# lorenzrichter/path-space-PDE-solver

Hardware: AMD Instinct MI355X
Metric: trajectory-timesteps/sec (K*N/s), d=100 HJB log-variance training iteration (higher is better)
Workload: dtype f32 (f16x3 split products: every matrix product as three f16 MFMAs, fp32 accumulate; state / sums fp32)

## Files before the change

### path-space-pde-solver_amd/csrc/hjb_kernels.h

```cpp
#pragma once
#include <cstdlib>
#include <type_traits>
#include <hip/hip_runtime.h>
#include <stdint.h>

namespace psp {

typedef float f32x4 __attribute__((ext_vector_type(4)));

struct HjbArgs {
    const float* params;
    const float* x0;
    const float* y0;
    const float* xi;
    float* path;
    float* D;
    float* XN;
    double* fwd_partial;
    const float* drift;
    const float* sigma;
    const float* runcost;
    const float* term;
    const double* sums;
    float* grad_partial;
// ... 91 lines not shown
    return addr;
}
template <class T>
__device__ __forceinline__ const T* opaque(const T* p) {
    return p + opaque_i(0);
}

#define PSP_PATH_STORE(ptr, val) __builtin_nontemporal_store((val), (ptr))

#ifndef PSP_PHILOX_ROUNDS
#define PSP_PHILOX_ROUNDS 7
#endif
constexpr int kPhiloxRounds = PSP_PHILOX_ROUNDS;
__device__ __forceinline__ void philox4x32_R(uint32_t c0, uint32_t c1, uint32_t c2, uint32_t c3,
                                             uint32_t k0, uint32_t k1, uint32_t (&out)[4]) {
#pragma unroll
    for (int r = 0; r < kPhiloxRounds; ++r) {
        const unsigned long long p0 = (unsigned long long)0xD2511F53u * (unsigned long long)c0;
        const unsigned long long p1 = (unsigned long long)0xCD9E8D57u * (unsigned long long)c2;
        const uint32_t hi0 = (uint32_t)(p0 >> 32), lo0 = (uint32_t)p0;
        const uint32_t hi1 = (uint32_t)(p1 >> 32), lo1 = (uint32_t)p1;
        const uint32_t n0 = __builtin_amdgcn_bitop3_b32(hi1, c1, k0, 0x96), n2 = __builtin_amdgcn_bitop3_b32(hi0, c3, k1, 0x96);
        c0 = n0; c1 = lo1; c2 = n2; c3 = lo0;
        k0 += 0x9E3779B9u; k1 += 0xBB67AE85u;
    }
    out[0] = c0; out[1] = c1; out[2] = c2; out[3] = c3;
}

__device__ __forceinline__ void philox_round(uint32_t& c0, uint32_t& c1, uint32_t& c2, uint32_t& c3, uint32_t k0, uint32_t k1) {
    const unsigned long long p0 = (unsigned long long)0xD2511F53u * (unsigned long long)c0;
    const unsigned long long p1 = (unsigned long long)0xCD9E8D57u * (unsigned long long)c2;
    const uint32_t hi0 = (uint32_t)(p0 >> 32), lo0 = (uint32_t)p0;
    const uint32_t hi1 = (uint32_t)(p1 >> 32), lo1 = (uint32_t)p1;
    const uint32_t n0 = __builtin_amdgcn_bitop3_b32(hi1, c1, k0, 0x96), n2 = __builtin_amdgcn_bitop3_b32(hi0, c3, k1, 0x96);
    c0 = n0; c1 = lo1; c2 = n2; c3 = lo0;
}

__device__ __forceinline__ f32x4 normal4(const uint32_t (&r)[4]) {
    const float s24 = 1.0f / 16777216.0f, h24 = 0.5f / 16777216.0f;
    const float u0 = __builtin_fmaf((float)(r[0] >> 8), s24, h24);
    const float u1 = __builtin_fmaf((float)(r[1] >> 8), s24, h24);
    const float u2 = __builtin_fmaf((float)(r[2] >> 8), s24, h24);
    const float u3 = __builtin_fmaf((float)(r[3] >> 8), s24, h24);
    const float ra = __builtin_amdgcn_sqrtf(-1.3862943611198906f * __builtin_amdgcn_logf(u0));
    const float rb = __builtin_amdgcn_sqrtf(-1.3862943611198906f * __builtin_amdgcn_logf(u2));
    f32x4 z;
    z[0] = ra * __builtin_amdgcn_cosf(u1);
    z[1] = ra * __builtin_amdgcn_sinf(u1);
    z[2] = rb * __builtin_amdgcn_cosf(u3);
    z[3] = rb * __builtin_amdgcn_sinf(u3);
    return z;
}

__device__ __forceinline__ f32x4 philox_block(uint32_t kglob, uint32_t step, uint32_t idx, uint32_t iter,
                                              uint32_t seed_lo, uint32_t seed_hi) {
    uint32_t r[4];
    philox4x32_R(kglob, step, idx, iter, seed_lo, seed_hi, r);
    return normal4(r);
}

template <int D, int DB>
__device__ __forceinline__ void regen_xi(f32x4 (&xin)[DB], uint32_t kglob, uint32_t n, int q, uint32_t iter,
                                         uint32_t seed_lo, uint32_t seed_hi) {
#pragma unroll
    for (int b = 0; b < DB; ++b) {
        xin[b] = philox_block(kglob, n, (uint32_t)(4 * b + q), iter, seed_lo, seed_hi);
        if (16 * b + 16 > D) {
#pragma unroll
            for (int r = 0; r < 4; ++r) if (16 * b + 4 * r + q >= D) xin[b][r] = 0.f;
        }
    }
}

template <class F>
__device__ __forceinline__ void stage_aop(float* dst, int MB, int KS, int tid, int nthr, F src) {
    const int total = MB * KS * 64;
    for (int idx = tid; idx < total; idx += nthr) {
        const int lane = idx & 63, t = idx >> 6;
        const int ks = t % KS, mb = t / KS;
        const int i = lane & 15, q = lane >> 4;
        dst[idx] = src(16 * mb + 4 * (i & 3) + (i >> 2), 4 * ks + q);
    }
}
template <class F>
__device__ __forceinline__ void stage_vec(float* dst, int NBLK, int tid, int nthr, F v) {
    for (int idx = tid; idx < NBLK * 16; idx += nthr) {
        const int r = idx & 3, q = (idx >> 2) & 3, b = idx >> 4;
        dst[idx] = v(16 * b + 4 * r + q);
    }
}

constexpr int kFenceMask = 0x1 | 0x2 | 0x4 | 0x10 | 0x20 | 0x40;
constexpr int kFenceAluOnly = 0x2 | 0x4;
template <int MB, int KS, int INB>
__device__ __forceinline__ void gemm_T(f32x4 (&acc)[MB], const float* wlds,
                                       const f32x4 (&in)[INB], int lane) {
    static_assert(INB * 4 >= KS, "input panel too small");
    static_assert(MB * KS * 256 <= 65536, "table exceeds the 16-bit ds_read immediate offset");
    constexpr int CH = (MB >= 4) ? 2 : 4;
    constexpr int NCH = cdiv(KS, CH);
    lane = opaque_i(lane);
    float buf[2][CH * MB];
#pragma unroll
    for (int kk = 0; kk < CH; ++kk)
#pragma unroll
        for (int mb = 0; mb < MB; ++mb)
// ... 159 lines not shown
#pragma unroll
            for (int e = 0; e < 8; ++e) {
                _Float16 h, l;
                split_f16(src(row, 32 * S + (e < 4 ? 4 * e : 16 + 4 * (e - 4)) + g), h, l);
                hi[e] = h; lo[e] = l;
            }
            f16x8* p = reinterpret_cast<f16x8*>(dstf + mb * SG::per_mb + S * 512);
            p[lane] = hi; p[64 + lane] = lo;
        }
    }
    if constexpr (SG::ODD) {
        for (int idx = tid; idx < MB * 64; idx += nthr) {
            const int lane = idx & 63, mb = idx >> 6;
            const int i = lane & 15, g = lane >> 4;
            const int row = 16 * mb + 4 * (i & 3) + (i >> 2);
            if constexpr (SG::ODD_F32) {
                dstf[mb * SG::per_mb + SG::NS * 512 + lane] = src(row, 32 * SG::NS + g);
            } else {
                f16x4 hi, lo;
#pragma unroll
                for (int e = 0; e < 4; ++e) {
                    _Float16 h, l;
                    split_f16(src(row, 32 * SG::NS + 4 * e + g), h, l);
                    hi[e] = h; lo[e] = l;
                }
                f16x4* p = reinterpret_cast<f16x4*>(dstf + mb * SG::per_mb + SG::NS * 512);
                p[lane] = hi; p[64 + lane] = lo;
            }
        }
    }
}
struct NoBetween { __device__ __forceinline__ void operator()(int) const {} };
template <int MB, int KS, int INB, int CU = 2, class BT = NoBetween>
__device__ __forceinline__ void gemm_Tx(f32x4 (&acc)[MB], const float* wlds, const f32x4 (&in)[INB], int lane, BT between = BT()) {
    constexpr int kFence = std::is_same<BT, NoBetween>::value ? kFenceMask : 0;
    using SG = SplitGeo<KS, INB>;
    constexpr int NS = SG::NS;
    static_assert(MB * SG::per_mb * 4 <= 65536, "table exceeds the 16-bit ds_read immediate offset");
    lane = opaque_i(lane);
    f32x4 corr[MB];
#pragma unroll
    for (int mb = 0; mb < MB; ++mb) corr[mb] = f32x4{0.f, 0.f, 0.f, 0.f};
    if constexpr (NS > 0) {
        const f16x8* tbl = reinterpret_cast<const f16x8*>(wlds) + lane;
        constexpr int NU = NS * MB, R = 2 * CU, PF = R - 1;
        f16x8 ah[R], al[R];
#pragma unroll
        for (int u = 0; u < PF; ++u)
            if (u < NU) {
                ah[u % R] = tbl[((u % MB) * SG::per_mb + (u / MB) * 512) / 4];
                al[u % R] = tbl[((u % MB) * SG::per_mb + (u / MB) * 512) / 4 + 64];
            }
        f16x8 bh, bl;
#pragma unroll
        for (int u = 0; u < NU; ++u) {
            if (u + PF < NU) {
                const int v = u + PF;
                ah[v % R] = tbl[((v % MB) * SG::per_mb + (v / MB) * 512) / 4];
                al[v % R] = tbl[((v % MB) * SG::per_mb + (v / MB) * 512) / 4 + 64];
            }
            const int S = u / MB, mb = u % MB;
            if (mb == 0) split8(in[2 * S], in[2 * S + 1], bh, bl);
            acc[mb] = __builtin_amdgcn_mfma_f32_16x16x32_f16(ah[u % R], bh, acc[mb], 0, 0, 0);
            corr[mb] = __builtin_amdgcn_mfma_f32_16x16x32_f16(ah[u % R], bl, corr[mb], 0, 0, 0);
            corr[mb] = __builtin_amdgcn_mfma_f32_16x16x32_f16(al[u % R], bh, corr[mb], 0, 0, 0);
            between(u);
            __builtin_amdgcn_sched_barrier(kFence);
        }
    }
    if constexpr (SG::ODD_F32) {
        const float bop = in[INB - 1][0];
#pragma unroll
        for (int mb = 0; mb < MB; ++mb) acc[mb] = mfma16(wlds[mb * SG::per_mb + NS * 512 + lane], bop, acc[mb]);
    }
    if constexpr (SG::ODD_H16) {
        f16x4 bh, bl;
        split4c(in[INB - 1], bh, bl);
#pragma unroll
        for (int mb = 0; mb < MB; ++mb) {
            const f16x4* p = reinterpret_cast<const f16x4*>(wlds + mb * SG::per_mb + NS * 512) + lane;
            const f16x4 a_hi = p[0], a_lo = p[64];
            acc[mb] = __builtin_amdgcn_mfma_f32_16x16x16f16(a_hi, bh, acc[mb], 0, 0, 0);
            corr[mb] = __builtin_amdgcn_mfma_f32_16x16x16f16(a_hi, bl, corr[mb], 0, 0, 0);
            corr[mb] = __builtin_amdgcn_mfma_f32_16x16x16f16(a_lo, bh, corr[mb], 0, 0, 0);
        }
    }
#pragma unroll
    for (int mb = 0; mb < MB; ++mb) acc[mb] = acc[mb] + kSplitInv * corr[mb];
}

template <int INB>
__device__ __forceinline__ void split_panel8(const f32x4 (&in)[INB], f16x8 (&bh)[INB / 2 > 0 ? INB / 2 : 1], f16x8 (&bl)[INB / 2 > 0 ? INB / 2 : 1]) {
#pragma unroll
    for (int S = 0; S < INB / 2; ++S) split8(in[2 * S], in[2 * S + 1], bh[S], bl[S]);
}
template <int MB, int KS, int INB, int CU = 2, class BT = NoBetween>
__device__ __forceinline__ void gemm_Txs(f32x4 (&acc)[MB], const float* wlds, const f16x8 (&bh)[INB / 2 > 0 ? INB / 2 : 1],
                                         const f16x8 (&bl)[INB / 2 > 0 ? INB / 2 : 1], const f32x4& last, int lane, BT between = BT()) {
    constexpr int kFence = std::is_same<BT, NoBetween>::value ? kFenceMask : 0;
    using SG = SplitGeo<KS, INB>;
    constexpr int NS = SG::NS;
    lane = opaque_i(lane);
    f32x4 corr[MB];
#pragma unroll
    for (int mb = 0; mb < MB; ++mb) corr[mb] = f32x4{0.f, 0.f, 0.f, 0.f};
    if constexpr (NS > 0) {
        const f16x8* tbl = reinterpret_cast<const f16x8*>(wlds) + lane;
        constexpr int NU = NS * MB, R = 2 * CU, PF = R - 1;
        f16x8 ah[R], al[R];
#pragma unroll
        for (int u = 0; u < PF; ++u)
            if (u < NU) {
                ah[u % R] = tbl[((u % MB) * SG::per_mb + (u / MB) * 512) / 4];
                al[u % R] = tbl[((u % MB) * SG::per_mb + (u / MB) * 512) / 4 + 64];
            }
#pragma unroll
        for (int u = 0; u < NU; ++u) {
            if (u + PF < NU) {
                const int v = u + PF;
                ah[v % R] = tbl[((v % MB) * SG::per_mb + (v / MB) * 512) / 4];
                al[v % R] = tbl[((v % MB) * SG::per_mb + (v / MB) * 512) / 4 + 64];
            }
            const int S = u / MB, mb = u % MB;
            acc[mb] = __builtin_amdgcn_mfma_f32_16x16x32_f16(ah[u % R], bh[S], acc[mb], 0, 0, 0);
            corr[mb] = __builtin_amdgcn_mfma_f32_16x16x32_f16(ah[u % R], bl[S], corr[mb], 0, 0, 0);
            corr[mb] = __builtin_amdgcn_mfma_f32_16x16x32_f16(al[u % R], bh[S], corr[mb], 0, 0, 0);
            between(u);
            __builtin_amdgcn_sched_barrier(kFence);
        }
    }
    if constexpr (SG::ODD_F32) {
        const float bop = last[0];
#pragma unroll
        for (int mb = 0; mb < MB; ++mb) acc[mb] = mfma16(wlds[mb * SG::per_mb + NS * 512 + lane], bop, acc[mb]);
    }
    if constexpr (SG::ODD_H16) {
        f16x4 b4h, b4l;
        split4c(last, b4h, b4l);
#pragma unroll
        for (int mb = 0; mb < MB; ++mb) {
            const f16x4* p = reinterpret_cast<const f16x4*>(wlds + mb * SG::per_mb + NS * 512) + lane;
            const f16x4 a_hi = p[0], a_lo = p[64];
            acc[mb] = __builtin_amdgcn_mfma_f32_16x16x16f16(a_hi, b4h, acc[mb], 0, 0, 0);
            corr[mb] = __builtin_amdgcn_mfma_f32_16x16x16f16(a_hi, b4l, corr[mb], 0, 0, 0);
            corr[mb] = __builtin_amdgcn_mfma_f32_16x16x16f16(a_lo, b4h, corr[mb], 0, 0, 0);
        }
    }
#pragma unroll
    for (int mb = 0; mb < MB; ++mb) acc[mb] = acc[mb] + kSplitInv * corr[mb];
}

__device__ __forceinline__ float qsum(float v) {
    v += __shfl_xor(v, 16);
    v += __shfl_xor(v, 32);
    return v;
}
__device__ __forceinline__ float jsumf(float v) {
    v += __shfl_xor(v, 1);
    v += __shfl_xor(v, 2);
    v += __shfl_xor(v, 4);
    v += __shfl_xor(v, 8);
    return v;
}
__device__ __forceinline__ double jsum(double v) {
    v += __shfl_xor(v, 1);
    v += __shfl_xor(v, 2);
    v += __shfl_xor(v, 4);
    v += __shfl_xor(v, 8);
    return v;
}

__device__ __forceinline__ float tanh_f32(float x) {
    const float e = __builtin_amdgcn_exp2f(fabsf(x) * 2.8853900817779268f);
    const float big = fmaf(-2.0f, __builtin_amdgcn_rcpf(e + 1.0f), 1.0f);
    return copysignf(big, x);
}
__device__ __forceinline__ f32x4 tanh4(f32x4 v) {
    f32x4 o;
    o[0] = tanh_f32(v[0]); o[1] = tanh_f32(v[1]); o[2] = tanh_f32(v[2]); o[3] = tanh_f32(v[3]);
    return o;
}
// ... 104 lines not shown
    const int k = t16 * 16 + j;
    const bool kvalid = wave_valid && k < a.K_local;
    const uint32_t kglob = (uint32_t)(a.k_offset + k);
    const float dt = a.dt, sqdt = a.sqdt;

    const float store_cxi = SPEC ? 1.f : ((k_store == 3) ? 0.f : 1.f);
    const float store_cz = SPEC ? 0.f : ((k_store == 3) ? 1.f : (k_store == 2 ? -a.sqdt : (k_adaptive ? 0.f : a.sqdt)));
    const bool do_store = FAST ? true : (k_store != 0);
    double sD = 0.0, sD2 = 0.0;
    if (wave_valid) {
        const f32x4* vecs0 = reinterpret_cast<const f32x4*>(lds + VEC) + q;
        const f32x4* vterm = vecs0 + (G::vterm - G::fVec) / 4;

        f32x4 X[DB];
#pragma unroll
        for (int b = 0; b < DB; ++b) {
#pragma unroll
            for (int r = 0; r < 4; ++r) {
                const int f = 16 * b + 4 * r + q;
                const float v = a.x0[(size_t)(kvalid ? k : 0) * a.x0_stride + (f < D ? f : D - 1)];
                X[b][r] = (f < D && kvalid) ? v : 0.f;
            }
        }
        float Y = a.y0 ? a.y0[0] : 0.f;
        float Fsum = 0.f, ULsum = 0.f;
#ifdef PSP_STAMPS
        unsigned long long stamps[8] = {0, 0, 0, 0, 0, 0, 0, 0};
#endif

        for (int n = 0; n < a.N; ++n) {
            PSP_STAMP(fs0);
            float tn = (float)n * dt;
            if constexpr (!FAST) { if (a.tfeat) tn = a.tfeat[n]; }
            const f32x4* vecs = opaque(vecs0);
            const f32x4* vb1 = vecs + (G::vb1 - G::fVec) / 4;
            const f32x4* vw1t = vecs + (G::vw1t - G::fVec) / 4;
            const f32x4* vb2 = vecs + (G::vb2 - G::fVec) / 4;
            const f32x4* vb3 = vecs + (G::vb3 - G::fVec) / 4;
            const f32x4* vdr = vecs + (G::vdr - G::fVec) / 4;
            const f32x4* vrun = vecs + (G::vrun - G::fVec) / 4;
            float* pblk = a.path + ((size_t)n * a.ntile16 + t16) * (size_t)G::PB + lane;
            auto x_store = [&](int u, int NU) __attribute__((always_inline)) {
                if (do_store) {
#pragma unroll
                    for (int ks = 0; ks < 4 * DB; ++ks)
                        if (ks >= u * (4 * DB) / NU && ks < (u + 1) * (4 * DB) / NU)
                            PSP_PATH_STORE(pblk + (G::pX / 64 + ks) * 64, X[ks >> 2][ks & 3]);
                }
            };
            if (!X3 && do_store) {
#pragma unroll
                for (int ks = 0; ks < 4 * DB; ++ks) PSP_PATH_STORE(pblk + (G::pX / 64 + ks) * 64, X[ks >> 2][ks & 3]);
            }
            f32x4 h1[HB];
#pragma unroll
            for (int m = 0; m < HB; ++m) h1[m] = vb1[m * 4] + tn * vw1t[m * 4];
            f32x4 Tn[DB];
            const bool early_drift = X3 && k_drift == DRIFT_DENSE;
            if constexpr (X3) {
                if (k_drift == DRIFT_DENSE) {
                    f16x8 xh[DB / 2 > 0 ? DB / 2 : 1], xl[DB / 2 > 0 ? DB / 2 : 1];
                    constexpr int NU1 = (DB / 2) * HB, NU2 = (DB / 2) * DB;
                    split_panel8<DB>(X, xh, xl);
                    gemm_Txs<HB, KSD, DB, 2>(h1, lds + oW1, xh, xl, X[DB - 1], lane, [&](int u) __attribute__((always_inline)) { x_store(u, NU1 + NU2); });
#pragma unroll
                    for (int b = 0; b < DB; ++b) Tn[b] = X[b];
                    gemm_Txs<DB, KSD, DB, 2>(Tn, ldsA, xh, xl, X[DB - 1], lane, [&](int u) __attribute__((always_inline)) { x_store(NU1 + u, NU1 + NU2); });
                    if constexpr (NU1 + NU2 == 0) x_store(0, 1);
                } else {
                    constexpr int NU1 = (DB / 2) * HB;
                    gemm_Tx<HB, KSD, DB, 2>(h1, lds + oW1, X, lane, [&](int u) __attribute__((always_inline)) { x_store(u, NU1); });
                    if constexpr (NU1 == 0) x_store(0, 1);
                }
            }
            else if constexpr (BF16) gemm_Tb<HB, DB>(h1, lds + oW1, X, lane);
            else gemm_T<HB, KSD, DB>(h1, lds + oW1, X, lane);
            PSP_STAMP(fs1);
#pragma unroll
            for (int m = 0; m < HB; ++m) h1[m] = tanh4(h1[m]);
            PSP_STAMP(fs2);
            f32x4 h2[HB];
#pragma unroll
            for (int m = 0; m < HB; ++m) h2[m] = vb2[m * 4];
            constexpr int NUH2 = (HB / 2) * HB, NUH3 = (HB / 2) * DB;
            constexpr bool PREGEN = X3 && FAST && (NUH2 + NUH3 > 0);
            [[maybe_unused]] f32x4 xig[PREGEN ? DB : 1];
            [[maybe_unused]] uint32_t pc0 = 0, pc1 = 0, pc2 = 0, pc3 = 0;
            constexpr int NSPC = kPhiloxRounds + 1;
            auto philox_slice = [&](int sidx) __attribute__((always_inline)) {
                const int b = sidx / NSPC, sub = sidx % NSPC;
                if (sub == 0) { pc0 = kglob; pc1 = (uint32_t)n; pc2 = (uint32_t)(4 * b + q); pc3 = iter_now; }
                if (sub < kPhiloxRounds) {
                    philox_round(pc0, pc1, pc2, pc3, a.seed_lo + (uint32_t)sub * 0x9E3779B9u, a.seed_hi + (uint32_t)sub * 0xBB67AE85u);
                    asm volatile("" : "+v"(pc0), "+v"(pc1), "+v"(pc2), "+v"(pc3));
                } else {
                    const uint32_t rr[4] = {pc0, pc1, pc2, pc3};
                    f32x4 xi = normal4(rr);
                    if (16 * b + 16 > D) {
#pragma unroll
                        for (int r = 0; r < 4; ++r) if (16 * b + 4 * r + q >= D) xi[r] = 0.f;
                    }
                    asm volatile("" : "+v"(xi));
                    xig[b < DB ? b : 0] = xi;
                }
            };
            auto philox_portion = [&](int u) __attribute__((always_inline)) {
                if constexpr (PREGEN) {
#pragma unroll
                    for (int sidx = 0; sidx < NSPC * DB; ++sidx)
                        if (sidx >= u * (NSPC * DB) / (NUH2 + NUH3) && sidx < (u + 1) * (NSPC * DB) / (NUH2 + NUH3)) philox_slice(sidx);
                }
            };
            auto h_store = [&](const f32x4 (&h)[HB], int slot, int u, int NU) __attribute__((always_inline)) {
                if (do_store) {
#pragma unroll
                    for (int ks = 0; ks < 4 * HB; ++ks)
                        if (ks >= u * (4 * HB) / NU && ks < (u + 1) * (4 * HB) / NU)
                            PSP_PATH_STORE(pblk + (slot / 64 + ks) * 64, h[ks >> 2][ks & 3]);
                }
            };
            if constexpr (X3) {
                gemm_Tx<HB, KSH, HB, 2>(h2, lds + oW2, h1, lane, [&](int u) __attribute__((always_inline)) { h_store(h1, G::pH1, u, NUH2); philox_portion(u); });
                if constexpr (NUH2 == 0) h_store(h1, G::pH1, 0, 1);
            }
            else if constexpr (BF16) gemm_Tb<HB, HB>(h2, lds + oW2, h1, lane);
            else gemm_T<HB, KSH, HB>(h2, lds + oW2, h1, lane);
#pragma unroll
            for (int m = 0; m < HB; ++m) h2[m] = tanh4(h2[m]);
            if (!X3 && do_store) {
#pragma unroll
                for (int ks = 0; ks < 4 * HB; ++ks) {
                    PSP_PATH_STORE(pblk + (G::pH1 / 64 + ks) * 64, h1[ks >> 2][ks & 3]);
                    PSP_PATH_STORE(pblk + (G::pH2 / 64 + ks) * 64, h2[ks >> 2][ks & 3]);
                }
            }
            f32x4 Z[DB];
#pragma unroll
            for (int m = 0; m < DB; ++m) Z[m] = vb3[m * 4];
            if constexpr (X3) {
                gemm_Tx<DB, KSH, HB, 2>(Z, lds + oW3, h2, lane, [&](int u) __attribute__((always_inline)) { h_store(h2, G::pH2, u, NUH3); philox_portion(NUH2 + u); });
                if constexpr (NUH3 == 0) h_store(h2, G::pH2, 0, 1);
            }
            else if constexpr (BF16) gemm_Tb<DB, HB>(Z, lds + oW3, h2, lane);
            else gemm_T<DB, KSH, HB>(Z, lds + oW3, h2, lane);
            PSP_STAMP(fs3);

            float S = 0.f, Pz = 0.f, UL = 0.f;
#pragma unroll
            for (int b = 0; b < DB; ++b) {
                f32x4 xi;
                if constexpr (PREGEN) {
                    xi = xig[b];
                } else if (FAST || a.noise_mode == NOISE_PHILOX) {
                    xi = philox_block(kglob, (uint32_t)n, (uint32_t)(4 * b + q), iter_now, a.seed_lo, a.seed_hi);
                } else {
                    const float* xrow = a.xi + ((size_t)(n + 1) * a.K_local + (kvalid ? k : 0)) * D;
#pragma unroll
                    for (int r = 0; r < 4; ++r) {
                        const int f = 16 * b + 4 * r + q;
                        const float v = xrow[f < D ? f : D - 1];
                        xi[r] = (f < D && kvalid) ? v : 0.f;
                    }
                }
                if (16 * b + 16 > D) {
#pragma unroll
                    for (int r = 0; r < 4; ++r) if (16 * b + 4 * r + q >= D) xi[r] = 0.f;
                }
                if (do_store && k_store != 4) {
                    const f32x4 wv = store_cxi * xi + store_cz * Z[b];
#pragma unroll
                    for (int r = 0; r < 4; ++r) PSP_PATH_STORE(pblk + (G::pXi / 64 + 4 * b + r) * 64, wv[r]);
                }
#pragma unroll
                for (int r = 0; r < 4; ++r) {
                    S = fmaf(Z[b][r], Z[b][r], S);
                    Pz = fmaf(Z[b][r], xi[r], Pz);
                }
                if (!FAST && a.uref) {
                    const float* ur = a.uref + (size_t)n * D;
#pragma unroll
                    for (int r = 0; r < 4; ++r) {
                        const int f = 16 * b + 4 * r + q;
                        const float e = (f < D) ? Z[b][r] + ur[f < D ? f : D - 1] : 0.f;
                        UL = fmaf(e, e, UL);
                    }
                }
                Z[b] = k_adaptive ? (sqdt * xi - dt * Z[b]) : (sqdt * xi);
            }
            ULsum = fmaf(UL, dt, ULsum);
            S = qsum(S);
            Pz = qsum(Pz);
            PSP_STAMP(fs4);

// ... 548 lines not shown
```

### path-space-pde-solver_amd/csrc/hjbx_kernels.h

```cpp
#pragma once
#include "hjb_kernels.h"

namespace psp {

template <int D, int H>
struct GeoX {
    using G = Geo<D, H>;
    static constexpr int DB = G::DB, HB = G::HB, KSD = G::KSD, KSH = G::KSH;
    static constexpr int T3 = 0, T2 = T3 + SplitGeo<KSD, DB>::floats(HB), EX = T2 + SplitGeo<KSH, HB>::floats(HB);
    static constexpr int hG = 0, hGl = hG + D * 32, hZ2 = hGl + D * 32, hZ2l = hZ2 + HB * 512, hZ1 = hZ2l + HB * 512,
                         hZ1l = hZ1 + HB * 512, PAIRH = hZ1l + HB * 512;
    static constexpr int RS = 16 * DB + 3 * 16 * HB;
    static constexpr int NX = cdiv(DB, 4);
    static constexpr int NT = DB + 2 * HB;
    static_assert(4 * RS <= 4 * (PAIRH / 2), "bias sums reuse the exchange area");
    static constexpr int GS = EX + 4 * (PAIRH / 2);
    static int lds_floats() { return GS + 12; }
};

template <int NB>
__device__ __forceinline__ void split_panel(const f32x4 (&v)[NB], f16x4 (&hi)[NB], f16x4 (&lo)[NB]) {
#pragma unroll
    for (int b = 0; b < NB; ++b) {
        if ((NB & 1) && b == NB - 1) split4c(v[b], hi[b], lo[b]);
// ... 84 lines not shown
    const float meanD = (a.loss_kind == LOSS_LOGVAR) ? (float)(a.sums[0] * invK) : 0.f;
    const float coef = (float)(2.0 * invK);
    {
        float wm = 0.f;
        for (int k = tid; k < a.K_local; k += nthr) {
            const float dk = a.D[k];
            wm = fmaxf(wm, fabsf(a.loss_kind == LOSS_WEIGHTS ? dk : coef * (dk - meanD)));
        }
#pragma unroll
        for (int o = 1; o < 64; o <<= 1) wm = fmaxf(wm, __shfl_xor(wm, o));
        if (lane == 0) lds[X::GS + 4 + wave] = wm;
    }
    stage_aop_x3<KSD, DB>(lds + X::T3, HB, tid, nthr, [&](int row, int col) {
        return (row < H && col < D) ? P[G::oW3 + col * H + row] : 0.f; });
    stage_aop_x3<KSH, HB>(lds + X::T2, HB, tid, nthr, [&](int row, int col) {
        return (row < H && col < H) ? P[G::oW2 + col * H + row] : 0.f; });
    __syncthreads();
    _Float16* exh = reinterpret_cast<_Float16*>(lds + X::EX);
    const bool xi_image = a.adaptive != 0 && (a.store_path == 1 || a.store_path == 4);
    auto g_scale = [&](float& gs, float& ginv) __attribute__((always_inline)) {
        const float* slot = lds + X::GS;
        float imax = fmaxf(fmaxf(slot[0], slot[1]), fmaxf(slot[2], slot[3]));
        if (xi_image || !(imax >= 1.1754944e-38f)) imax = xi_image ? 8.0f : 1.0f;
        const float wmax = fmaxf(fmaxf(fmaxf(slot[4], slot[5]), fmaxf(slot[6], slot[7])),
                                 fmaxf(fmaxf(slot[8], slot[9]), fmaxf(slot[10], slot[11])));
        const float amax = wmax * a.sqdt * imax;
        const unsigned e = (__float_as_uint(amax) >> 23) & 0xFFu;
        const bool ok = e >= 1u && e <= 253u;
        gs = ok ? __uint_as_float((254u - e) << 23) : 1.0f;
        ginv = ok ? __uint_as_float(e << 23) : 1.0f;
    };
    const f32x4 zero4 = {0.f, 0.f, 0.f, 0.f};
    const float sqdt = a.sqdt, dt = a.dt;
    constexpr bool regen = REGEN;
    const uint32_t iter_now = a.iter_dev ? *a.iter_dev : a.iter;
    const long long nblk = (long long)a.N * a.ntile16;
    const long long nround = (nblk + 3) / 4;
    const int R = (int)((nround - blockIdx.x + gridDim.x - 1) / gridDim.x);

    if (producer) {
        f32x4 sG[DB], sZ2[HB], sZ1[HB], sT1[HB];
#pragma unroll
        for (int b = 0; b < DB; ++b) sG[b] = zero4;
#pragma unroll
        for (int m = 0; m < HB; ++m) { sZ2[m] = zero4; sZ1[m] = zero4; sT1[m] = zero4; }
        auto own_block = [&](int it2) __attribute__((always_inline)) {
            const long long b0 = ((long long)blockIdx.x + (long long)it2 * gridDim.x) * 4 + sub;
            return b0 < nblk ? b0 : -1LL;
        };
        auto path_of = [&](int it2) __attribute__((always_inline)) {
            const long long b0 = own_block(it2);
            return a.path + (size_t)(b0 >= 0 ? b0 : nblk - 1) * (size_t)G::PB + lane;
        };
        f32x4 xin[DB], h2n[HB], h1n[HB];
        float dkn;
        {
            const long long b0 = own_block(0);
            const long long blk = b0 >= 0 ? b0 : nblk - 1;
            const float* pb = path_of(0);
            const int k0 = (int)(blk % a.ntile16) * 16 + j;
            dkn = a.D[k0 < a.K_local ? k0 : 0];
            if constexpr (regen) {
#pragma unroll
                for (int b = 0; b < DB; ++b) xin[b] = zero4;
            } else {
#pragma unroll
                for (int b = 0; b < DB; ++b)
#pragma unroll
                    for (int r = 0; r < 4; ++r) xin[b][r] = pb[G::pXi + (4 * b + r) * 64];
            }
            if constexpr (regen) {
#pragma unroll
                for (int m = 0; m < HB; ++m)
#pragma unroll
                    for (int r = 0; r < 4; ++r) h2n[m][r] = pb[G::pH2 + (4 * m + r) * 64];
#pragma unroll
                for (int m = 0; m < HB; ++m)
#pragma unroll
                    for (int r = 0; r < 4; ++r) h1n[m][r] = pb[G::pH1 + (4 * m + r) * 64];
            }
        }
        float gs, ginv;
        {
            const long long b0 = own_block(0);
            const int k0 = (int)((b0 >= 0 ? b0 : nblk - 1) % a.ntile16) * 16 + j;
            const bool kv = b0 >= 0 && k0 < a.K_local;
            float am = 0.f;
#pragma unroll
            for (int b = 0; b < DB; ++b)
#pragma unroll
                for (int r = 0; r < 4; ++r) am = fmaxf(am, kv ? fabsf(xin[b][r]) : 0.f);
#pragma unroll
            for (int o = 1; o < 64; o <<= 1) am = fmaxf(am, __shfl_xor(am, o));
            if (lane == 0) lds[X::GS + sub] = am;
            __syncthreads();
            g_scale(gs, ginv);
        }
#ifdef PSP_STAMPS
        unsigned long long stamps[8] = {0, 0, 0, 0, 0, 0, 0, 0};
#endif
        for (int it = 0; it <= R; ++it) {
            PSP_STAMP(tp0);
            if (it < R) {
                const long long blk0 = own_block(it);
                const bool bvalid = blk0 >= 0;
                const long long blk = bvalid ? blk0 : nblk - 1;
                const int t16 = (int)(blk % a.ntile16);
                const int k = t16 * 16 + j;
                const bool kvalid = bvalid && k < a.K_local;
                const float tn = (float)(blk / a.ntile16) * dt;
                _Float16* ex0 = exh + ((it & 1) * 2 + (sub >> 1)) * PAIRH + (sub & 1) * 4 + (j & 3);
                _Float16* exr[4] = {ex0 + (((j >> 2) ^ 0) * 8), ex0 + (((j >> 2) ^ 1) * 8), ex0 + (((j >> 2) ^ 2) * 8), ex0 + (((j >> 2) ^ 3) * 8)};
                const float* pn = path_of(it + 1);
                const float* pc = path_of(it);
                const float dkc = dkn;
                if constexpr (!regen) {
#pragma unroll
                    for (int m = 0; m < HB; ++m)
#pragma unroll
                        for (int r = 0; r < 4; ++r) h2n[m][r] = pc[G::pH2 + (4 * m + r) * 64];
                }
                const float wk = kvalid ? (a.loss_kind == LOSS_WEIGHTS ? dkc : coef * (dkc - meanD)) : 0.f;
                f32x4 Gt[DB];
                if constexpr (regen) {
                    const uint32_t kg = (uint32_t)(a.k_offset + k), nstep = (uint32_t)(blk / a.ntile16);
                    const int qo = opaque_i(q);
#pragma unroll
                    for (int b = 0; b < DB; ++b) {
                        f32x4 xi = philox_block(kg, nstep, (uint32_t)(4 * b + qo), iter_now, a.seed_lo, a.seed_hi);
                        if (16 * b + 16 > D) {
#pragma unroll
                            for (int r = 0; r < 4; ++r) if (16 * b + 4 * r + q >= D) xi[r] = 0.f;
                        }
                        {
#pragma clang fp contract(off)
                            Gt[b] = (wk * sqdt * gs) * xi;
                            sG[b] += Gt[b];
                        }
                        __builtin_amdgcn_sched_barrier(0);
                    }
                } else {
                    {
#pragma clang fp contract(off)
#pragma unroll
                        for (int b = 0; b < DB; ++b) {
                            Gt[b] = (wk * sqdt * gs) * xin[b];
                            sG[b] += Gt[b];
                        }
                    }
                }
                PSP_STAMP(tp1);
                PSP_ACC(0, tp1, tp0);
                f16x4 Gh[DB], Gl[DB];
                split_panel<DB>(Gt, Gh, Gl);
#pragma unroll
                for (int b = 0; b < DB; ++b)
#pragma unroll
                    for (int r = 0; r < 4; ++r) {
                        const int f = 16 * b + 4 * r + q;
                        if (16 * b + 16 <= D || f < D) {
                            exr[r][X::hG + f * 32] = Gh[b][r];
                            exr[r][X::hGl + f * 32] = Gl[b][r];
                        }
                    }
                PSP_STAMP(tp2);
                PSP_ACC(1, tp2, tp1);
                f32x4 dz2[HB];
#pragma unroll
                for (int m = 0; m < HB; ++m) dz2[m] = zero4;
                gemm_Txp<HB, KSD, DB>(dz2, lds + X::T3, Gh, Gl, Gt[DB - 1][0], lane);
                {
#pragma clang fp contract(off)
#pragma unroll
                    for (int m = 0; m < HB; ++m) { dz2[m] = dz2[m] * (1.0f - h2n[m] * h2n[m]); sZ2[m] += dz2[m]; }
                }
                if constexpr (regen) {
                    __builtin_amdgcn_sched_barrier(0);
#pragma unroll
                    for (int m = 0; m < HB; ++m)
#pragma unroll
                        for (int r = 0; r < 4; ++r) h2n[m][r] = pn[G::pH2 + (4 * m + r) * 64];
                } else {
#pragma unroll
                    for (int m = 0; m < HB; ++m)
#pragma unroll
                        for (int r = 0; r < 4; ++r) h1n[m][r] = pc[G::pH1 + (4 * m + r) * 64];
                    const long long n0 = own_block(it + 1);
                    const long long nb1 = n0 >= 0 ? n0 : nblk - 1;
                    const int k1 = (int)(nb1 % a.ntile16) * 16 + j;
                    dkn = a.D[k1 < a.K_local ? k1 : 0];
#pragma unroll
                    for (int b = 0; b < DB; ++b)
#pragma unroll
                        for (int r = 0; r < 4; ++r) xin[b][r] = pn[G::pXi + (4 * b + r) * 64];
                }
                PSP_STAMP(tp3);
                PSP_ACC(2, tp3, tp2);
                f16x4 Zh[HB], Zl[HB];
                split_panel<HB>(dz2, Zh, Zl);
#pragma unroll
                for (int m = 0; m < HB; ++m)
#pragma unroll
                    for (int r = 0; r < 4; ++r) {
                        exr[r][X::hZ2 + (16 * m + 4 * r + q) * 32] = Zh[m][r];
                        exr[r][X::hZ2l + (16 * m + 4 * r + q) * 32] = Zl[m][r];
                    }
                f32x4 dz1[HB];
#pragma unroll
                for (int m = 0; m < HB; ++m) dz1[m] = zero4;
                gemm_Txp<HB, KSH, HB>(dz1, lds + X::T2, Zh, Zl, dz2[HB - 1][0], lane);
                {
#pragma clang fp contract(off)
#pragma unroll
                    for (int m = 0; m < HB; ++m) {
                        dz1[m] = dz1[m] * (1.0f - h1n[m] * h1n[m]);
                        sZ1[m] += dz1[m];
                        sT1[m] += tn * dz1[m];
                    }
                }
                if constexpr (regen) {
                    __builtin_amdgcn_sched_barrier(0);
                    const long long n0 = own_block(it + 1);
                    const long long nb1 = n0 >= 0 ? n0 : nblk - 1;
                    const int k1 = (int)(nb1 % a.ntile16) * 16 + j;
                    dkn = a.D[k1 < a.K_local ? k1 : 0];
#pragma unroll
                    for (int m = 0; m < HB; ++m)
#pragma unroll
                        for (int r = 0; r < 4; ++r) h1n[m][r] = pn[G::pH1 + (4 * m + r) * 64];
                }
                split_panel<HB>(dz1, Zh, Zl);
#pragma unroll
                for (int m = 0; m < HB; ++m)
#pragma unroll
                    for (int r = 0; r < 4; ++r) {
                        exr[r][X::hZ1 + (16 * m + 4 * r + q) * 32] = Zh[m][r];
                        exr[r][X::hZ1l + (16 * m + 4 * r + q) * 32] = Zl[m][r];
                    }
            }
            PSP_STAMP(tp4);
            PSP_ACC(3, tp4, tp0);
            __syncthreads();
            PSP_STAMP(tp5);
            PSP_ACC(4, tp5, tp4);
            PSP_ACC(6, tp5, tp0);
        }
#ifdef PSP_STAMPS
        if (a.dbg && lane == 0) {
            stamps[7] = (unsigned long long)R;
            for (int i = 0; i < 8; ++i) a.dbg[((size_t)blockIdx.x * 8 + wave) * 8 + i] = stamps[i];
        }
#endif
        float* red = lds + X::EX + sub * RS;
#pragma unroll
        for (int b = 0; b < DB; ++b)
#pragma unroll
            for (int r = 0; r < 4; ++r) {
                const float v = ginv * jsumf(sG[b][r]);
                if (j == 0) red[16 * b + 4 * r + q] = v;
            }
#pragma unroll
        for (int m = 0; m < HB; ++m)
#pragma unroll
            for (int r = 0; r < 4; ++r) {
                const float v2 = ginv * jsumf(sZ2[m][r]), v1 = ginv * jsumf(sZ1[m][r]), vt = ginv * jsumf(sT1[m][r]);
                if (j == 0) {
                    red[16 * DB + 16 * m + 4 * r + q] = v2;
                    red[16 * DB + 16 * HB + 16 * m + 4 * r + q] = v1;
                    red[16 * DB + 32 * HB + 16 * m + 4 * r + q] = vt;
                }
            }
        __syncthreads();
        return;
    }
    const int ibw = sub < HB ? sub : HB - 1;
    int obx[NX];
#pragma unroll
    for (int s = 0; s < NX; ++s) obx[s] = (sub + 4 * s) < DB ? (sub + 4 * s) : DB - 1;
    f32x4 a3[DB], a2[HB], a1[HB][NX], c1[HB][NX];
#pragma unroll
    for (int b = 0; b < DB; ++b) a3[b] = zero4;
#pragma unroll
    for (int m = 0; m < HB; ++m) {
        a2[m] = zero4;
#pragma unroll
        for (int s = 0; s < NX; ++s) { a1[m][s] = zero4; c1[m][s] = zero4; }
    }
    const int nblk_i = (int)nblk;
    auto blk_at = [&](long long c0) __attribute__((always_inline)) {
        const int c = (c0 < (long long)nblk_i) ? (int)c0 : nblk_i - 1;
        return __builtin_amdgcn_readfirstlane(c);
// ... 180 lines not shown
```

Baseline: 1.632 billion.

## Spread Philox normal generation across GEMM units with cost-weighted slices

The in-kernel Philox RNG regeneration is split into finer slices: the Box-Muller finish is broken into six separately scheduled pieces, and slices are assigned to MFMA units by a compile-time cost model. Interleaving now also covers the first-layer GEMMs in the speculative path, not just the later layers. The intent is to hide transcendental and integer work under MFMA latency more evenly. Separately, the backward kernel replaces per-iteration 64-bit div/mod of the block index with an incrementally advanced step/tile counter pair, removing costly integer division. This adds compile-time complexity and more register pressure from the new lambdas, and the cost weights are hand-tuned.

```diff
diff --git a/path-space-pde-solver_amd/csrc/hjb_kernels.h b/path-space-pde-solver_amd/csrc/hjb_kernels.h
--- a/path-space-pde-solver_amd/csrc/hjb_kernels.h
+++ b/path-space-pde-solver_amd/csrc/hjb_kernels.h
@@ -167,6 +167,18 @@
     return z;
 }
 
+constexpr int kPhiloxSlices = kPhiloxRounds + 6;
+__host__ __device__ constexpr int philox_slice_cost_before(int sub) {
+    const int k = sub - kPhiloxRounds;
+    return sub <= kPhiloxRounds ? 12 * sub : 12 * kPhiloxRounds + (k <= 2 ? 18 * k : (k <= 4 ? 36 + 13 * (k - 2) : 62 + 16 * (k - 4)));
+}
+__host__ __device__ constexpr int philox_slice_unit(int sidx, int ncall, int NUT) {
+    const int call = philox_slice_cost_before(kPhiloxSlices);
+    const int b = sidx / kPhiloxSlices, sub = sidx % kPhiloxSlices;
+    const int lo = b * call + philox_slice_cost_before(sub), hi = b * call + philox_slice_cost_before(sub + 1);
+    return (lo + hi) * NUT / (2 * call * ncall);
+}
+
 __device__ __forceinline__ f32x4 philox_block(uint32_t kglob, uint32_t step, uint32_t idx, uint32_t iter,
                                               uint32_t seed_lo, uint32_t seed_hi) {
     uint32_t r[4];
@@ -432,8 +444,8 @@
                 al[u % R] = tbl[((u % MB) * SG::per_mb + (u / MB) * 512) / 4 + 64];
             }
         f16x8 bh, bl;
-#pragma unroll
-        for (int u = 0; u < NU; ++u) {
+        auto unit = [&](auto uc) __attribute__((always_inline)) {
+            const int u = uc;
             if (u + PF < NU) {
                 const int v = u + PF;
                 ah[v % R] = tbl[((v % MB) * SG::per_mb + (v / MB) * 512) / 4];
@@ -444,8 +456,14 @@
             acc[mb] = __builtin_amdgcn_mfma_f32_16x16x32_f16(ah[u % R], bh, acc[mb], 0, 0, 0);
             corr[mb] = __builtin_amdgcn_mfma_f32_16x16x32_f16(ah[u % R], bl, corr[mb], 0, 0, 0);
             corr[mb] = __builtin_amdgcn_mfma_f32_16x16x32_f16(al[u % R], bh, corr[mb], 0, 0, 0);
-            between(u);
+            between(uc);
             __builtin_amdgcn_sched_barrier(kFence);
+        };
+        if constexpr (std::is_same<BT, NoBetween>::value) {
+#pragma unroll
+            for (int u = 0; u < NU; ++u) unit(u);
+        } else {
+            static_for<0, NU>(unit);
         }
     }
     if constexpr (SG::ODD_F32) {
@@ -494,8 +512,8 @@
                 ah[u % R] = tbl[((u % MB) * SG::per_mb + (u / MB) * 512) / 4];
                 al[u % R] = tbl[((u % MB) * SG::per_mb + (u / MB) * 512) / 4 + 64];
             }
-#pragma unroll
-        for (int u = 0; u < NU; ++u) {
+        auto unit = [&](auto uc) __attribute__((always_inline)) {
+            const int u = uc;
             if (u + PF < NU) {
                 const int v = u + PF;
                 ah[v % R] = tbl[((v % MB) * SG::per_mb + (v / MB) * 512) / 4];
@@ -505,8 +523,14 @@
             acc[mb] = __builtin_amdgcn_mfma_f32_16x16x32_f16(ah[u % R], bh[S], acc[mb], 0, 0, 0);
             corr[mb] = __builtin_amdgcn_mfma_f32_16x16x32_f16(ah[u % R], bl[S], corr[mb], 0, 0, 0);
             corr[mb] = __builtin_amdgcn_mfma_f32_16x16x32_f16(al[u % R], bh[S], corr[mb], 0, 0, 0);
-            between(u);
+            between(uc);
             __builtin_amdgcn_sched_barrier(kFence);
+        };
+        if constexpr (std::is_same<BT, NoBetween>::value) {
+#pragma unroll
+            for (int u = 0; u < NU; ++u) unit(u);
+        } else {
+            static_for<0, NU>(unit);
         }
     }
     if constexpr (SG::ODD_F32) {
@@ -717,6 +741,55 @@
 #pragma unroll
                 for (int ks = 0; ks < 4 * DB; ++ks) PSP_PATH_STORE(pblk + (G::pX / 64 + ks) * 64, X[ks >> 2][ks & 3]);
             }
+            constexpr int NUH2 = (HB / 2) * HB, NUH3 = (HB / 2) * DB;
+            constexpr bool PREGEN = X3 && FAST && (NUH2 + NUH3 > 0);
+            constexpr int NUE = SPEC ? (DB / 2) * HB + (DB / 2) * DB : 0;
+            constexpr int NUT = NUE + NUH2 + NUH3;
+            [[maybe_unused]] f32x4 xig[PREGEN ? DB : 1];
+            [[maybe_unused]] uint32_t pc0 = 0, pc1 = 0, pc2 = 0, pc3 = 0;
+            [[maybe_unused]] float pf0 = 0.f, pf1 = 0.f, pf2 = 0.f, pf3 = 0.f;
+            auto philox_slice = [&](int sidx) __attribute__((always_inline)) {
+                const int b = sidx / kPhiloxSlices, sub = sidx % kPhiloxSlices, fin = sub - kPhiloxRounds;
+                const float s24 = 1.0f / 16777216.0f, h24 = 0.5f / 16777216.0f;
+                if (sub == 0) { pc0 = kglob; pc1 = (uint32_t)n; pc2 = (uint32_t)(4 * b + q); pc3 = iter_now; }
+                if (sub < kPhiloxRounds) {
+                    philox_round(pc0, pc1, pc2, pc3, a.seed_lo + (uint32_t)sub * 0x9E3779B9u, a.seed_hi + (uint32_t)sub * 0xBB67AE85u);
+                    asm volatile("" : "+v"(pc0), "+v"(pc1), "+v"(pc2), "+v"(pc3));
+                } else if (fin == 0) {
+                    pf0 = __builtin_fmaf((float)(pc0 >> 8), s24, h24);
+                    pf1 = __builtin_fmaf((float)(pc1 >> 8), s24, h24);
+                    asm volatile("" : "+v"(pf0), "+v"(pf1));
+                } else if (fin == 1) {
+                    pf2 = __builtin_fmaf((float)(pc2 >> 8), s24, h24);
+                    pf3 = __builtin_fmaf((float)(pc3 >> 8), s24, h24);
+                    asm volatile("" : "+v"(pf2), "+v"(pf3));
+                } else if (fin == 2) {
+                    pf0 = __builtin_amdgcn_sqrtf(-1.3862943611198906f * __builtin_amdgcn_logf(pf0));
+                    asm volatile("" : "+v"(pf0));
+                } else if (fin == 3) {
+                    pf2 = __builtin_amdgcn_sqrtf(-1.3862943611198906f * __builtin_amdgcn_logf(pf2));
+                    asm volatile("" : "+v"(pf2));
+                } else {
+                    const int r0 = fin == 4 ? 0 : 2;
+                    const float rad = fin == 4 ? pf0 : pf2, ang = fin == 4 ? pf1 : pf3;
+                    float z0 = rad * __builtin_amdgcn_cosf(ang), z1 = rad * __builtin_amdgcn_sinf(ang);
+                    if (16 * b + 16 > D) {
+                        if (16 * b + 4 * r0 + q >= D) z0 = 0.f;
+                        if (16 * b + 4 * (r0 + 1) + q >= D) z1 = 0.f;
+                    }
+                    asm volatile("" : "+v"(z0), "+v"(z1));
+                    xig[b < DB ? b : 0][r0] = z0;
+                    xig[b < DB ? b : 0][r0 + 1] = z1;
+                }
+            };
+            auto philox_portion = [&](auto uc) __attribute__((always_inline)) {
+                if constexpr (PREGEN) {
+                    static_for<0, kPhiloxSlices * DB>([&](auto sc) __attribute__((always_inline)) {
+                        constexpr int sidx = decltype(sc)::value, u = decltype(uc)::value;
+                        if constexpr (philox_slice_unit(sidx, DB, NUT) == u) philox_slice(sidx);
+                    });
+                }
+            };
             f32x4 h1[HB];
 #pragma unroll
             for (int m = 0; m < HB; ++m) h1[m] = vb1[m * 4] + tn * vw1t[m * 4];
@@ -727,10 +800,10 @@
                     f16x8 xh[DB / 2 > 0 ? DB / 2 : 1], xl[DB / 2 > 0 ? DB / 2 : 1];
                     constexpr int NU1 = (DB / 2) * HB, NU2 = (DB / 2) * DB;
                     split_panel8<DB>(X, xh, xl);
-                    gemm_Txs<HB, KSD, DB, 2>(h1, lds + oW1, xh, xl, X[DB - 1], lane, [&](int u) __attribute__((always_inline)) { x_store(u, NU1 + NU2); });
+                    gemm_Txs<HB, KSD, DB, 2>(h1, lds + oW1, xh, xl, X[DB - 1], lane, [&](auto uc) __attribute__((always_inline)) { x_store(uc, NU1 + NU2); if constexpr (SPEC) philox_portion(uc); });
 #pragma unroll
                     for (int b = 0; b < DB; ++b) Tn[b] = X[b];
-                    gemm_Txs<DB, KSD, DB, 2>(Tn, ldsA, xh, xl, X[DB - 1], lane, [&](int u) __attribute__((always_inline)) { x_store(NU1 + u, NU1 + NU2); });
+                    gemm_Txs<DB, KSD, DB, 2>(Tn, ldsA, xh, xl, X[DB - 1], lane, [&](auto uc) __attribute__((always_inline)) { x_store(NU1 + uc, NU1 + NU2); if constexpr (SPEC) philox_portion(std::integral_constant<int, NU1 + decltype(uc)::value>{}); });
                     if constexpr (NU1 + NU2 == 0) x_store(0, 1);
                 } else {
                     constexpr int NU1 = (DB / 2) * HB;
@@ -747,35 +820,6 @@
             f32x4 h2[HB];
 #pragma unroll
             for (int m = 0; m < HB; ++m) h2[m] = vb2[m * 4];
-            constexpr int NUH2 = (HB / 2) * HB, NUH3 = (HB / 2) * DB;
-            constexpr bool PREGEN = X3 && FAST && (NUH2 + NUH3 > 0);
-            [[maybe_unused]] f32x4 xig[PREGEN ? DB : 1];
-            [[maybe_unused]] uint32_t pc0 = 0, pc1 = 0, pc2 = 0, pc3 = 0;
-            constexpr int NSPC = kPhiloxRounds + 1;
-            auto philox_slice = [&](int sidx) __attribute__((always_inline)) {
-                const int b = sidx / NSPC, sub = sidx % NSPC;
-                if (sub == 0) { pc0 = kglob; pc1 = (uint32_t)n; pc2 = (uint32_t)(4 * b + q); pc3 = iter_now; }
-                if (sub < kPhiloxRounds) {
-                    philox_round(pc0, pc1, pc2, pc3, a.seed_lo + (uint32_t)sub * 0x9E3779B9u, a.seed_hi + (uint32_t)sub * 0xBB67AE85u);
-                    asm volatile("" : "+v"(pc0), "+v"(pc1), "+v"(pc2), "+v"(pc3));
-                } else {
-                    const uint32_t rr[4] = {pc0, pc1, pc2, pc3};
-                    f32x4 xi = normal4(rr);
-                    if (16 * b + 16 > D) {
-#pragma unroll
-                        for (int r = 0; r < 4; ++r) if (16 * b + 4 * r + q >= D) xi[r] = 0.f;
-                    }
-                    asm volatile("" : "+v"(xi));
-                    xig[b < DB ? b : 0] = xi;
-                }
-            };
-            auto philox_portion = [&](int u) __attribute__((always_inline)) {
-                if constexpr (PREGEN) {
-#pragma unroll
-                    for (int sidx = 0; sidx < NSPC * DB; ++sidx)
-                        if (sidx >= u * (NSPC * DB) / (NUH2 + NUH3) && sidx < (u + 1) * (NSPC * DB) / (NUH2 + NUH3)) philox_slice(sidx);
-                }
-            };
             auto h_store = [&](const f32x4 (&h)[HB], int slot, int u, int NU) __attribute__((always_inline)) {
                 if (do_store) {
 #pragma unroll
@@ -785,7 +829,7 @@
                 }
             };
             if constexpr (X3) {
-                gemm_Tx<HB, KSH, HB, 2>(h2, lds + oW2, h1, lane, [&](int u) __attribute__((always_inline)) { h_store(h1, G::pH1, u, NUH2); philox_portion(u); });
+                gemm_Tx<HB, KSH, HB, 2>(h2, lds + oW2, h1, lane, [&](auto uc) __attribute__((always_inline)) { h_store(h1, G::pH1, uc, NUH2); philox_portion(std::integral_constant<int, NUE + decltype(uc)::value>{}); });
                 if constexpr (NUH2 == 0) h_store(h1, G::pH1, 0, 1);
             }
             else if constexpr (BF16) gemm_Tb<HB, HB>(h2, lds + oW2, h1, lane);
@@ -803,7 +847,7 @@
 #pragma unroll
             for (int m = 0; m < DB; ++m) Z[m] = vb3[m * 4];
             if constexpr (X3) {
-                gemm_Tx<DB, KSH, HB, 2>(Z, lds + oW3, h2, lane, [&](int u) __attribute__((always_inline)) { h_store(h2, G::pH2, u, NUH3); philox_portion(NUH2 + u); });
+                gemm_Tx<DB, KSH, HB, 2>(Z, lds + oW3, h2, lane, [&](auto uc) __attribute__((always_inline)) { h_store(h2, G::pH2, uc, NUH3); philox_portion(std::integral_constant<int, NUE + NUH2 + decltype(uc)::value>{}); });
                 if constexpr (NUH3 == 0) h_store(h2, G::pH2, 0, 1);
             }
             else if constexpr (BF16) gemm_Tb<DB, HB>(Z, lds + oW3, h2, lane);
diff --git a/path-space-pde-solver_amd/csrc/hjbx_kernels.h b/path-space-pde-solver_amd/csrc/hjbx_kernels.h
--- a/path-space-pde-solver_amd/csrc/hjbx_kernels.h
+++ b/path-space-pde-solver_amd/csrc/hjbx_kernels.h
@@ -160,13 +160,21 @@
             const long long b0 = own_block(it2);
             return a.path + (size_t)(b0 >= 0 ? b0 : nblk - 1) * (size_t)G::PB + lane;
         };
+        const long long rstride = 4LL * gridDim.x;
+        const int inc_s = (int)(rstride / a.ntile16), inc_t = (int)(rstride % a.ntile16);
+        auto advance = [&](int& s_, int& t_) __attribute__((always_inline)) {
+            s_ += inc_s; t_ += inc_t;
+            if (t_ >= a.ntile16) { t_ -= a.ntile16; ++s_; }
+        };
+        int sc = (int)(((long long)blockIdx.x * 4 + sub) / a.ntile16), tc = (int)(((long long)blockIdx.x * 4 + sub) % a.ntile16);
+        int sn = sc, tn1 = tc;
+        advance(sn, tn1);
         f32x4 xin[DB], h2n[HB], h1n[HB];
         float dkn;
         {
             const long long b0 = own_block(0);
-            const long long blk = b0 >= 0 ? b0 : nblk - 1;
             const float* pb = path_of(0);
-            const int k0 = (int)(blk % a.ntile16) * 16 + j;
+            const int k0 = (b0 >= 0 ? tc : a.ntile16 - 1) * 16 + j;
             dkn = a.D[k0 < a.K_local ? k0 : 0];
             if constexpr (regen) {
 #pragma unroll
@@ -191,7 +199,7 @@
         float gs, ginv;
         {
             const long long b0 = own_block(0);
-            const int k0 = (int)((b0 >= 0 ? b0 : nblk - 1) % a.ntile16) * 16 + j;
+            const int k0 = (b0 >= 0 ? tc : a.ntile16 - 1) * 16 + j;
             const bool kv = b0 >= 0 && k0 < a.K_local;
             float am = 0.f;
 #pragma unroll
@@ -212,11 +220,10 @@
             if (it < R) {
                 const long long blk0 = own_block(it);
                 const bool bvalid = blk0 >= 0;
-                const long long blk = bvalid ? blk0 : nblk - 1;
-                const int t16 = (int)(blk % a.ntile16);
+                const int t16 = bvalid ? tc : a.ntile16 - 1, step = bvalid ? sc : a.N - 1;
                 const int k = t16 * 16 + j;
                 const bool kvalid = bvalid && k < a.K_local;
-                const float tn = (float)(blk / a.ntile16) * dt;
+                const float tn = (float)step * dt;
                 _Float16* ex0 = exh + ((it & 1) * 2 + (sub >> 1)) * PAIRH + (sub & 1) * 4 + (j & 3);
                 _Float16* exr[4] = {ex0 + (((j >> 2) ^ 0) * 8), ex0 + (((j >> 2) ^ 1) * 8), ex0 + (((j >> 2) ^ 2) * 8), ex0 + (((j >> 2) ^ 3) * 8)};
                 const float* pn = path_of(it + 1);
@@ -231,7 +238,7 @@
                 const float wk = kvalid ? (a.loss_kind == LOSS_WEIGHTS ? dkc : coef * (dkc - meanD)) : 0.f;
                 f32x4 Gt[DB];
                 if constexpr (regen) {
-                    const uint32_t kg = (uint32_t)(a.k_offset + k), nstep = (uint32_t)(blk / a.ntile16);
+                    const uint32_t kg = (uint32_t)(a.k_offset + k), nstep = (uint32_t)step;
                     const int qo = opaque_i(q);
 #pragma unroll
                     for (int b = 0; b < DB; ++b) {
@@ -293,9 +300,7 @@
                     for (int m = 0; m < HB; ++m)
 #pragma unroll
                         for (int r = 0; r < 4; ++r) h1n[m][r] = pc[G::pH1 + (4 * m + r) * 64];
-                    const long long n0 = own_block(it + 1);
-                    const long long nb1 = n0 >= 0 ? n0 : nblk - 1;
-                    const int k1 = (int)(nb1 % a.ntile16) * 16 + j;
+                    const int k1 = (own_block(it + 1) >= 0 ? tn1 : a.ntile16 - 1) * 16 + j;
                     dkn = a.D[k1 < a.K_local ? k1 : 0];
 #pragma unroll
                     for (int b = 0; b < DB; ++b)
@@ -328,9 +333,7 @@
                 }
                 if constexpr (regen) {
                     __builtin_amdgcn_sched_barrier(0);
-                    const long long n0 = own_block(it + 1);
-                    const long long nb1 = n0 >= 0 ? n0 : nblk - 1;
-                    const int k1 = (int)(nb1 % a.ntile16) * 16 + j;
+                    const int k1 = (own_block(it + 1) >= 0 ? tn1 : a.ntile16 - 1) * 16 + j;
                     dkn = a.D[k1 < a.K_local ? k1 : 0];
 #pragma unroll
                     for (int m = 0; m < HB; ++m)
@@ -345,6 +348,8 @@
                         exr[r][X::hZ1 + (16 * m + 4 * r + q) * 32] = Zh[m][r];
                         exr[r][X::hZ1l + (16 * m + 4 * r + q) * 32] = Zl[m][r];
                     }
+                sc = sn; tc = tn1;
+                advance(sn, tn1);
             }
             PSP_STAMP(tp4);
             PSP_ACC(3, tp4, tp0);
```

New measurement: 1.642 billion (median of 6 runs). No clear change (+0.6%).
